# nekStab/nekStab_next

Measured on AMD Instinct MI355X. Metric: Arnoldi-step GB/s (achieved HBM) + Ritz-value rel-err, N=1e8 m=128, higher is better.
Workload: dtype f64

## Files before the change

### include/nekkrylov.h

```cpp
#ifndef NEKKRYLOV_H
#define NEKKRYLOV_H

#include <stddef.h>
#include <stdint.h>

#ifdef __cplusplus
extern "C" {
#endif

#define NKV_ABI_VERSION 3

#define NKV_TILE 4096
#define NKV_MAX_COLS 1024
#define NKV_ROT_MAX_OUT 256

#define NKV_OK 0
#define NKV_EINVAL 1
#define NKV_EHIP 2
#define NKV_ENAN 3
#define NKV_ESHAPE 4
#define NKV_ECALLBACK 5
#define NKV_EBREAKDOWN 6

#define NKV_TIME 0x1u
// ... 50 lines not shown
                     double* f, double* nrm2_dev, void* ws, unsigned flags, void* stream);
int nkv_block_update_dot(const nkv_layout* L, const double* w, const double* Q, int j, const double* h_dev,
                         double* f, double* hout_dev, void* ws, unsigned flags, void* stream);
int nkv_arnoldi_finish(const nkv_layout* L, const double* f, const double* nrm2_dev, double* q_out,
                       int j, const double* h1_dev, const double* h2_dev, double* hcol_dev,
                       unsigned flags, void* stream);

int nkv_combine(const nkv_layout* L, const double* Q, int k, const double* y_dev, double* out, unsigned flags,
                void* stream);
int nkv_normalize_store(const nkv_layout* L, const double* f, const double* nrm2_dev, double* q_next,
                        double* beta_dev, unsigned flags, void* stream);
int nkv_mgs2_step(const nkv_layout* L, const double* w, const double* Q, int j, double* f, double* q_out,
                  double* hcol_dev, void* ws, unsigned flags, void* stream);
int nkv_axpy_dot(const nkv_layout* L, const double* w, double* f, const double* alpha_dev, const double* qa,
                 const double* qb, double* out_dev, void* ws, unsigned flags, void* stream);

int nkv_block_dot2(const nkv_layout* L, const double* w, const double* Q, int j, const double* x,
                   const double* y, double* h_dev, void* ws, unsigned flags, void* stream);
int nkv_dcgs2_coef(int m, const double* hq_dev, const double* hw_dev, const double* nrm_prev_dev, double* H_dev,
                   int64_t ldh, double* coef_dev, void* ws, void* stream);
int nkv_dcgs2_update(const nkv_layout* L, const double* w, const double* Q, int m, const double* coef_dev,
                     double* qj, const double* win, double* fout, double* nrm2_dev, void* ws, unsigned flags,
                     void* stream);

int nkv_mgs_icwy_solve(int j, double* G, int64_t ldg, const double* grow, const double* b, double* x,
                       void* stream);

int nkv_gkl_coef(int side, int m, const double* hq_dev, const double* hw_dev, double* M_dev, int64_t ldm,
                 double* A_self, double* r_self, const double* A_other, const double* r_other, int64_t lda,
                 double* coef_dev, void* ws, void* stream);

typedef int (*nkv_matvec_fn)(void* user, const double* x, double* y, void* stream);
typedef int (*nkv_allreduce_fn)(void* user, double* buf, int n, void* stream);
size_t nkv_arnoldi_scratch_doubles(int m);
int nkv_arnoldi_dcgs2(const nkv_layout* L, const double* w, double* Q, int mstart, int mend, double* H_dev,
                      int64_t ldh, double* f, double* scratch_dev, void* ws, nkv_matvec_fn matvec, void* mv_user,
                      nkv_allreduce_fn allreduce, void* ar_user, unsigned flags, void* stream);

int nkv_gmres_dcgs2(const nkv_layout* L, const double* w, double* Q, int kmax, double beta, double tol2,
                    double* H_dev, int64_t ldh, double* f, double* scratch_dev, void* ws, nkv_matvec_fn matvec,
                    void* mv_user, nkv_allreduce_fn allreduce, void* ar_user, double* res_hist, int* k_out,
                    unsigned flags, void* stream);

int nkv_update_hessenberg(const nkv_layout* L, const double* w, const double* Q, int j, double* f, double* q_out,
                          double* hcol_dev, double* scratch_dev, void* ws, nkv_allreduce_fn allreduce, void* ar_user,
                          unsigned flags, void* stream);
// ... 4 lines not shown

int nkv_rotate(const nkv_layout* L, double* Q, int k, const double* V_dev, int ldv, void* stream);

int nkv_rotate_cols(const nkv_layout* L, double* Q, int k, const double* V_dev, int ldv, int n_out,
                    void* stream);

#define NKV_ROT_PATH_FEW 1
#define NKV_ROT_PATH_WIDE 2
#define NKV_ROT_PATH_STREAM 3
#define NKV_ROT_PATH_CHUNKED 4
int nkv_rotate_plan(const nkv_layout* L, int k, int ldv, int n_out, int* path, int* inst, int* wg_threads,
                    int* rows_per_tile);

#define NKV_STREAM_BLOCK_DOT 1
#define NKV_STREAM_BLOCK_UPDATE 2
#define NKV_STREAM_UPDATE_DOT 3
#define NKV_STREAM_BLOCK_DOT2 4
#define NKV_STREAM_DCGS2_UPDATE 5
#define NKV_STREAM_AXPY_DOT 6
#define NKV_STREAM_BLAS1 7
#define NKV_STREAM_OP_DIAG 8
#define NKV_STREAM_FINISH 9
#define NKV_STREAM_SPLIT 10
#define NKV_STREAM_LOOP_TILES 1
#define NKV_STREAM_LOOP_UNITS 2
typedef struct nkv_plan {
    int64_t kernel, pairs, nw, cpw, wg_threads, rows_per_tile, tiles, grid_x, grid_y, launches, band_tiles,
        last_grid_x, work_loop, units, fields_per_block, partial_slots, partial_cols;
} nkv_plan;
int nkv_stream_plan(const nkv_layout* L, int op, int j, unsigned flags, nkv_plan* plan);

int nkv_op_diag(const nkv_layout* L, const double* d, const double* x, double* y, double time_scale,
                void* stream);
int nkv_op_rot2(const nkv_layout* L, const double* c, const double* s, const double* d_rest,
                const double* x, double* y, int transpose, void* stream);
int nkv_op_cdiag(const nkv_layout* L, const double* cr, const double* ci, const double* x, double* y, int conj,
                 void* stream);

int nkv_wavemaker(const nkv_layout* L, const double* dRe, const double* dIm, const double* aRe, const double* aIm,
                  double* out, int ncomp, void* stream);
int nkv_gradm1(const nkv_layout* L, int lx1, int ldim, const double* D, const double* xm, const double* ym,
               const double* zm, const double* u, int nfld, int64_t u_stride, double* grad, int64_t g_stride,
               void* stream);
int nkv_bf_sensitivity(const nkv_layout* L, const double* dRe, const double* dIm, const double* aRe,
                       const double* aIm, const double* grad, double* out, int ncomp, void* stream);

// ... 149 lines not shown
```

### nekstab_next_amd/_lib.py

```python
from __future__ import annotations

import ctypes
import os
from ctypes import CFUNCTYPE, POINTER, Structure, c_char_p, c_double, c_int, c_int32, c_int64, c_size_t, c_uint, c_uint64, c_void_p

import torch

_HERE = os.path.dirname(os.path.abspath(__file__))
LIB_PATH = os.path.join(_HERE, "libnekkrylov.so")

NKV_ABI_VERSION = 3
NKV_TILE = 4096
NKV_MAX_COLS = 1024
NKV_ROT_MAX_OUT = 256
NKV_GS_MAX_FIELDS = 64
NKV_ROT_PATH_FEW, NKV_ROT_PATH_WIDE, NKV_ROT_PATH_STREAM, NKV_ROT_PATH_CHUNKED = 1, 2, 3, 4
(NKV_STREAM_BLOCK_DOT, NKV_STREAM_BLOCK_UPDATE, NKV_STREAM_UPDATE_DOT, NKV_STREAM_BLOCK_DOT2, NKV_STREAM_DCGS2_UPDATE,
 NKV_STREAM_AXPY_DOT, NKV_STREAM_BLAS1, NKV_STREAM_OP_DIAG, NKV_STREAM_FINISH, NKV_STREAM_SPLIT) = range(1, 11)
NKV_STREAM_LOOP_TILES, NKV_STREAM_LOOP_UNITS = 1, 2
NKV_OK, NKV_EINVAL, NKV_EHIP, NKV_ENAN, NKV_ESHAPE, NKV_ECALLBACK, NKV_EBREAKDOWN = 0, 1, 2, 3, 4, 5, 6
NKV_TIME = 0x1
NKV_ACCUMULATE = 0x2
NKV_OVERWRITE = 0x4
NKV_NORM2 = 0x8
NKV_TIME_DOT = 0x10
NKV_X_IS_LAST = 0x20
NKV_MGS2 = 0x40
NKV_MGS_ICWY = 0x100
NKV_MGS_LAGGED = 0x200
NKV_CHECK_BREAKDOWN = 0x80
NKV_SFD_MONITOR = 0x400
NKV_TDF_STORE = 0x800
NKV_BF_IMAG = 0x1000
NKV_BF_PERTURBATION = 0x2000
(NKV_VC_VORTICITY, NKV_VC_LAMBDA2, NKV_VC_Q, NKV_VC_DELTA, NKV_VC_SWIRLING, NKV_VC_OMEGA, NKV_VC_SYMMETRIC,
 NKV_VC_ASSYMETRIC, NKV_VC_LAMBDA_CI, NKV_VC_COUNT) = range(10)


class NkvError(RuntimeError):

    def __init__(self, code: int, where: str, msg: str):
        super().__init__(f"{where}: status {code}: {msg}")
# ... 35 lines not shown
_SIGNATURES = {
    "nkv_abi_version": (c_int, []),
    "nkv_layout_init": (c_int, [_L, c_int, c_int, c_int, c_int64, c_int64, c_int, c_int, c_int]),
    "nkv_last_error": (c_char_p, []),
    "nkv_device_info": (c_int, [POINTER(c_int), POINTER(c_int), POINTER(c_int64), c_char_p, c_int]),
    "nkv_workspace_bytes": (c_size_t, [_L, c_int]),
    "nkv_check_status": (c_int, [_P, _P]),
    "nkv_zero": (c_int, [_L, _P, c_uint, _P]),
    "nkv_copy": (c_int, [_L, _P, _P, c_uint, _P]),
    "nkv_scal": (c_int, [_L, _P, c_double, c_uint, _P]),
    "nkv_axpby": (c_int, [_L, _P, c_double, _P, c_double, c_uint, _P]),
    "nkv_sub3": (c_int, [_L, _P, _P, _P, c_uint, _P]),
    "nkv_axpy_dev": (c_int, [_L, _P, _P, c_double, _P, c_uint, _P]),
    "nkv_normalize_dev": (c_int, [_L, _P, _P, _P, c_uint, _P]),
    "nkv_dot": (c_int, [_L, _P, _P, _P, _P, _P, c_uint, _P]),
    "nkv_block_dot": (c_int, [_L, _P, _P, c_int, _P, _P, _P, c_uint, _P]),
    "nkv_block_update": (c_int, [_L, _P, _P, c_int, _P, _P, _P, _P, c_uint, _P]),
    "nkv_block_update_dot": (c_int, [_L, _P, _P, c_int, _P, _P, _P, _P, c_uint, _P]),
    "nkv_arnoldi_finish": (c_int, [_L, _P, _P, _P, c_int, _P, _P, _P, c_uint, _P]),
    "nkv_block_dot2": (c_int, [_L, _P, _P, c_int, _P, _P, _P, _P, c_uint, _P]),
    "nkv_dcgs2_coef": (c_int, [c_int, _P, _P, _P, _P, c_int64, _P, _P, _P]),
    "nkv_mgs_icwy_solve": (c_int, [c_int, _P, c_int64, _P, _P, _P, _P]),
    "nkv_dcgs2_update": (c_int, [_L, _P, _P, c_int, _P, _P, _P, _P, _P, _P, c_uint, _P]),
    "nkv_arnoldi_scratch_doubles": (c_size_t, [c_int]),
    "nkv_arnoldi_dcgs2": (c_int, [_L, _P, _P, c_int, c_int, _P, c_int64, _P, _P, _P, MATVEC_FN, _P, ALLREDUCE_FN, _P,
                                  c_uint, _P]),
    "nkv_update_hessenberg": (c_int, [_L, _P, _P, c_int, _P, _P, _P, _P, _P, ALLREDUCE_FN, _P, c_uint, _P]),
    "nkv_gmres_dcgs2": (c_int, [_L, _P, _P, c_int, c_double, c_double, _P, c_int64, _P, _P, _P, MATVEC_FN, _P,
                                ALLREDUCE_FN, _P, _P, _P, c_uint, _P]),
    "nkv_arnoldi_factorization": (c_int, [_L, _P, _P, c_int, c_int, _P, c_int64, _P, _P, _P, MATVEC_FN, _P,
                                          ALLREDUCE_FN, _P, c_uint, _P]),
    "nkv_combine": (c_int, [_L, _P, c_int, _P, _P, c_uint, _P]),
    "nkv_normalize_store": (c_int, [_L, _P, _P, _P, _P, c_uint, _P]),
    "nkv_mgs2_step": (c_int, [_L, _P, _P, c_int, _P, _P, _P, _P, c_uint, _P]),
    "nkv_axpy_dot": (c_int, [_L, _P, _P, _P, _P, _P, _P, _P, c_uint, _P]),
    "nkv_rotate": (c_int, [_L, _P, c_int, _P, c_int, _P]),
    "nkv_rotate_cols": (c_int, [_L, _P, c_int, _P, c_int, c_int, _P]),
    "nkv_rotate_plan": (c_int, [_L, c_int, c_int, c_int, POINTER(c_int), POINTER(c_int), POINTER(c_int),
                                POINTER(c_int)]),
    "nkv_stream_plan": (c_int, [_L, c_int, c_int, c_uint, POINTER(nkv_plan)]),
    "nkv_op_diag": (c_int, [_L, _P, _P, _P, c_double, _P]),
    "nkv_op_rot2": (c_int, [_L, _P, _P, _P, _P, _P, c_int, _P]),
    "nkv_op_cdiag": (c_int, [_L, _P, _P, _P, _P, c_int, _P]),
    "nkv_fill_hash": (c_int, [_L, _P, c_uint64, c_int64, c_int64, _P]),
    "nkv_mth_rand_add": (c_int, [_L, c_int, c_int, c_int, c_int64, _P, _P, _P, c_double, c_double, c_double, _P, _P]),
    "nkv_group_average": (c_int, [c_int64, _P, _P, _P, _P]),
# ... 110 lines not shown
```

### nekstab_next_amd/arnoldi.py

```python
from __future__ import annotations

import numpy as np
import torch

from . import _lib
from ._lib import NKV_NORM2, NKV_TIME, NKV_TIME_DOT, NKV_X_IS_LAST
from .operators import LinearOperator
from .vector import Basis, NekContext, NekVector


class HessenbergDev:

    def __init__(self, ctx: NekContext, k: int):
        self.ctx, self.k = ctx, k
        self.t = torch.zeros((k, k + 1), dtype=torch.float64, device=ctx.device)

    def col_ptr(self, c: int) -> int:
        return self.t[c].data_ptr()

    def download(self) -> np.ndarray:
        return np.asfortranarray(self.t.detach().cpu().numpy().T)

    def upload(self, H: np.ndarray) -> None:
        self.t.copy_(torch.as_tensor(np.ascontiguousarray(np.asarray(H, dtype=np.float64).T)).to(self.ctx.device))
# ... 60 lines not shown
    elif mode == "mgs2":
        ctx.call("nkv_dot", w, f.ptr, Q.col_ptr(0), h1[0:1].data_ptr(), ws, tf, st)
        ctx.comm.allreduce_(h1[0:1])
        fl = NKV_TIME | (NKV_TIME_DOT if tf else 0)
        for p, h in enumerate((h1, h2)):
            for i in range(j):
                last = i + 1 == j
                qn = Q.col_ptr(i + 1) if not last else (Q.col_ptr(0) if p == 0 else None)
                out = h[i + 1:i + 2] if not last else (h2[0:1] if p == 0 else nrm)
                ctx.call("nkv_axpy_dot", w, f.ptr, h[i:i + 1].data_ptr(), Q.col_ptr(i), qn, out.data_ptr(), ws, fl,
                         st)
                ctx.comm.allreduce_(out)
    else:
        raise ValueError(f"unknown orthogonalisation mode {mode!r}")
    if ctx.timer:
        ctx.timer.begin("finish")
    ctx.call("nkv_arnoldi_finish", f.ptr, nrm.data_ptr(), out_ptr, j, h1.data_ptr(), h2.data_ptr(),
             hcol_ptr, 0, st)
    if ctx.timer:
        ctx.timer.end("finish", 16.0 * ctx.layout.N)


def _dcgs2_step(ctx: NekContext, Q: Basis, Hd: HessenbergDev, j: int, f: NekVector, first: bool,
                nrm2: torch.Tensor | None = None) -> None:
    w, ws, st = ctx.w.data_ptr(), ctx.ws.data_ptr(), ctx.stream
    lay, tm = ctx.layout, ctx.timer
    tf = NKV_TIME if ctx.time_in_dot else 0
    m = j - 1
    h = ctx.hd[: 2 * j]
    hp, cp = h.data_ptr(), ctx.coef.data_ptr()
    u = Q.col_ptr(m)
    if tm:
        tm.begin("block_dot2")
    ctx.call("nkv_block_dot2", w, Q.ptr, j, u, f.ptr, hp, ws, tf | NKV_X_IS_LAST, st)
    if tm:
        tm.end("block_dot2", 8.0 * ((j - 1) * lay.N_w + 2 * lay.N_w + lay.n_v))
    ctx.comm.allreduce_(h)
    nprev = None if first else (nrm2.data_ptr() if nrm2 is not None else hp + 8 * m)
    ctx.call_nl("nkv_dcgs2_coef", m, hp, hp + 8 * j, nprev, Hd.t.data_ptr(), Hd.k + 1, cp, ws, st)
    if tm:
        tm.begin("dcgs2_update")
    ctx.call("nkv_dcgs2_update", w, Q.ptr, m, cp, u, f.ptr, Q.col_ptr(j), None if nrm2 is None else nrm2.data_ptr(),
             ws, NKV_TIME | (NKV_TIME_DOT if tf else 0), st)
    if tm:
        tm.end("dcgs2_update", 8.0 * (m * lay.N + 4 * lay.N) + (0.0 if nrm2 is None else 8.0 * lay.n_v))
    if nrm2 is not None:
        ctx.comm.allreduce_(nrm2)


def _dcgs2_close(ctx: NekContext, Q: Basis, Hd: HessenbergDev, m: int) -> None:
    w, ws, st = ctx.w.data_ptr(), ctx.ws.data_ptr(), ctx.stream
    lay, tm = ctx.layout, ctx.timer
    tf = NKV_TIME if ctx.time_in_dot else 0
    h, coef = ctx.hd[: m + 1], ctx.coef
    u = Q.col_ptr(m)
    if tm:
        tm.begin("block_dot")
    ctx.call("nkv_block_dot", w, Q.ptr, m + 1, u, h.data_ptr(), ws, tf, st)
    if tm:
        tm.end("block_dot", 8.0 * ((m + 1) * lay.N_w + lay.N_w + lay.n_v))
    ctx.comm.allreduce_(h)
    ctx.call_nl("nkv_dcgs2_coef", m, h.data_ptr(), None, h.data_ptr() + 8 * m, Hd.t.data_ptr(), Hd.k + 1,
                coef.data_ptr(), ws, st)
    if tm:
        tm.begin("block_update")
    ctx.call("nkv_block_update", w, Q.ptr, m, h.data_ptr(), u, None, ws, NKV_TIME, st)
    if tm:
        tm.end("block_update", 8.0 * (m * lay.N + 2 * lay.N))
    ctx.call("nkv_normalize_dev", u, coef[2 * m + 3:].data_ptr(), None, 0, st)


def _icwy_gram(ctx: NekContext, Q: Basis, mstart: int) -> torch.Tensor:
    ldg = ctx.max_cols + 1
    G = getattr(ctx, "_icwy_G", None)
    if G is None:
        G = ctx._icwy_G = torch.zeros((ldg, ldg), dtype=torch.float64, device=ctx.device)
    w, ws, st = ctx.w.data_ptr(), ctx.ws.data_ptr(), ctx.stream
    tf = NKV_TIME if ctx.time_in_dot else 0
    for i in range(1, mstart - 1):
        ctx.call("nkv_block_dot", w, Q.ptr, i, Q.col_ptr(i), G[i].data_ptr(), ws, tf, st)
        ctx.comm.allreduce_(G[i, :i])
    return G

# ... 174 lines not shown
        raise errors[0]
    _lib.check(rc, entry)


def arnoldi_factorization(ctx: NekContext, op: LinearOperator, Q: Basis, Hd: HessenbergDev, mstart: int,
                          mend: int, f: NekVector | None = None, mode: str = "cgs2", transpose: bool = False,
                          on_step=None) -> None:
    if mend < mstart:
        return
    if Q.k < mend + 1:
        raise ValueError("basis too small")
    if f is None:
        f = ctx.vector()
    if mode == "dcgs2-native":
        if on_step is None:
            if mend > ctx.max_cols or mend + 1 > Hd.k + 1:
                raise ValueError(f"step {mend} exceeds max_cols {ctx.max_cols} / H size {Hd.k}")
            _dcgs2_native(ctx, op, Q, Hd, mstart, mend, f, transpose)
            return
        mode = "dcgs2"
    if mode == "dcgs2" and on_step is not None:
        if mend > ctx.max_cols or mend + 1 > Hd.k + 1:
            raise ValueError(f"step {mend} exceeds max_cols {ctx.max_cols} / H size {Hd.k}")
        for mstep in range(mstart, mend + 1):
            (op.rmatvec if transpose else op.matvec)(Q[mstep - 1], f)
            _dcgs2_step(ctx, Q, Hd, mstep, f, first=(mstep == mstart))
            if mstep > mstart:
                on_step(mstep - 1)
        _dcgs2_close(ctx, Q, Hd, mend)
        on_step(mend)
        return
    if mode == "mgs2-lagged-native":
        if on_step is None:
            if mend > ctx.max_cols or mend + 1 > Hd.k + 1:
                raise ValueError(f"step {mend} exceeds max_cols {ctx.max_cols} / H size {Hd.k}")
            _dcgs2_native(ctx, op, Q, Hd, mstart, mend, f, transpose, entry="nkv_arnoldi_factorization",
                          flags=_lib.NKV_MGS_LAGGED)
            return
        mode = "mgs2-lagged"
    if mode == "mgs2-lagged":
        if mend > ctx.max_cols or mend + 1 > Hd.k + 1:
            raise ValueError(f"step {mend} exceeds max_cols {ctx.max_cols} / H size {Hd.k}")
        _lagged_factorization(ctx, op, Q, Hd, mstart, mend, f, transpose, on_step)
        return
    if mode == "mgs2-icwy-native":
        if on_step is None:
            if mend > ctx.max_cols or mend + 1 > Hd.k + 1:
                raise ValueError(f"step {mend} exceeds max_cols {ctx.max_cols} / H size {Hd.k}")
            _dcgs2_native(ctx, op, Q, Hd, mstart, mend, f, transpose, entry="nkv_arnoldi_factorization",
                          flags=_lib.NKV_MGS_ICWY)
            return
        mode = "mgs2-icwy"
    if mode == "mgs2-icwy":
        if mend > ctx.max_cols or mend + 1 > Hd.k + 1:
            raise ValueError(f"step {mend} exceeds max_cols {ctx.max_cols} / H size {Hd.k}")
        G = _icwy_gram(ctx, Q, mstart)
        for mstep in range(mstart, mend + 1):
            (op.rmatvec if transpose else op.matvec)(Q[mstep - 1], f)
            _icwy_step(ctx, Q, Hd, mstep, f, G)
            if on_step is not None:
                on_step(mstep)
        return
    if mode in ("cgs2-native", "mgs2-native") and on_step is None:
        if mend > ctx.max_cols or mend + 1 > Hd.k + 1:
            raise ValueError(f"step {mend} exceeds max_cols {ctx.max_cols} / H size {Hd.k}")
        _dcgs2_native(ctx, op, Q, Hd, mstart, mend, f, transpose, entry="nkv_arnoldi_factorization",
                      flags=_lib.NKV_MGS2 if mode == "mgs2-native" else 0)
        return
    if mode == "dcgs2" and on_step is None:
        if mend > ctx.max_cols or mend + 1 > Hd.k + 1:
            raise ValueError(f"step {mend} exceeds max_cols {ctx.max_cols} / H size {Hd.k}")
        for mstep in range(mstart, mend + 1):
            (op.rmatvec if transpose else op.matvec)(Q[mstep - 1], f)
            _dcgs2_step(ctx, Q, Hd, mstep, f, first=(mstep == mstart))
        _dcgs2_close(ctx, Q, Hd, mend)
        return
    if mode == "dcgs2":
        mode = "cgs2"
    for mstep in range(mstart, mend + 1):
        x = Q[mstep - 1]
        (op.rmatvec if transpose else op.matvec)(x, f)
        update_hessenberg_matrix(ctx, Q, mstep, f, Hd, mode)
        if on_step is not None:
            on_step(mstep)


class FactorizationGraph:

    def __init__(self, ctx: NekContext, op: LinearOperator, Q: Basis, Hd: HessenbergDev, f: NekVector,
                 mode: str = "cgs2"):
        self.ctx, self.op, self.Q, self.Hd, self.f, self.mode = ctx, op, Q, Hd, f, mode
        self.graphs = {}

    HOST_SYNC_MODES = ("mgs2-lagged", "mgs2-lagged-native")

    def usable(self) -> bool:
        return self.ctx.comm.world == 1 and self.mode not in self.HOST_SYNC_MODES

# ... 17 lines not shown
```

### nekstab_next_amd/csrc/core.hip

```cpp
#include "nkv_internal.h"

namespace nkvi {

thread_local char g_err[512] = "";

int fail(int code, const char* fmt, ...) {
    va_list ap;
    va_start(ap, fmt);
    vsnprintf(g_err, sizeof(g_err), fmt, ap);
    va_end(ap);
    return code;
}

int device_cus() {
    static int cus[64] = {0};
    int dev = 0;
    if (hipGetDevice(&dev) != hipSuccess || dev < 0 || dev >= 64) return 256;
    if (!cus[dev]) {
        int n = 0;
        cus[dev] = (hipDeviceGetAttribute(&n, hipDeviceAttributeMultiprocessorCount, dev) == hipSuccess && n > 0)
                       ? n : 256;
    }
    return cus[dev];
}
// ... 122 lines not shown
            if (bmax > kMaxBlocks) bmax = kMaxBlocks;
            p.grid_x = bmax / p.grid_y;
            if (p.grid_x > p.tiles) p.grid_x = p.tiles;
            if (p.grid_x < 1) p.grid_x = 1;
            p.work_loop = NKV_STREAM_LOOP_TILES;
            p.units = p.tiles;
            p.band_tiles = p.tiles > 0 ? p.tiles : 1;
            p.launches = p.tiles > 0 ? 1 : 0;
            p.last_grid_x = p.grid_x;
            p.partial_slots = p.tiles > 0 ? p.grid_x * p.grid_y : 0;
            p.partial_cols = two ? 2 * j : j;
            break;
        }
        case NKV_STREAM_BLOCK_UPDATE: {
            if (j < 0) return fail(NKV_EINVAL, "j=%d < 0", j);
            set_tile_grid(&p, L, large ? NKV_PAIRS : NKV_PAIRS_SMALL, j <= NKV_UPD_SMALL_J ? 4 * kMaxBlocks : kMaxBlocks);
            set_bands(&p, NKV_UPD_ROUNDS, true);
            if (flags & NKV_NORM2) {
                p.partial_slots = p.grid_x;
                p.partial_cols = 1;
            }
            break;
        }
        case NKV_STREAM_UPDATE_DOT: {
            if (j < 1 || j > NKV_MAX_COLS) return fail(NKV_EINVAL, "j=%d outside 1..%d", j, NKV_MAX_COLS);
            if (j > 256 || rows >= (int64_t)1 << 29) {
                p.kernel = NKV_STREAM_SPLIT;
                break;
            }
            constexpr int NW = NKV_FUSE_NW;
            p.nw = j <= NKV_FUSE_SMALL_J ? 4 : (j <= NW * 16 ? NW : 16);
            p.cpw = (j + p.nw - 1) / p.nw;
            p.pairs = 1;
            p.wg_threads = p.nw * 64;
            p.rows_per_tile = kFuseRows;
            p.tiles = rows / kFuseRows;
            const int64_t gcap = (j >= NKV_FUSE_MID_LO && j <= NKV_FUSE_MID_HI) ? NKV_FUSE_G_MID : NKV_FUSE_G;
            p.grid_x = p.tiles < gcap ? p.tiles : gcap;
            if (p.grid_x < 1) p.grid_x = 1;
            p.grid_y = 1;
            p.work_loop = NKV_STREAM_LOOP_TILES;
            p.units = p.tiles;
            p.fields_per_block = 1;
            set_bands(&p, NKV_FUSE_ROUNDS, true);
            p.partial_slots = p.grid_x;
            p.partial_cols = j;
            break;
        }
        case NKV_STREAM_DCGS2_UPDATE: {
            if (j < 0) return fail(NKV_EINVAL, "m=%d < 0", j);
            set_tile_grid(&p, L, large ? NKV_DC_PAIRS : NKV_PAIRS_SMALL, NKV_DC_G < kMaxBlocks ? NKV_DC_G : kMaxBlocks);
            if (!(flags & NKV_NORM2)) {
                set_bands(&p, NKV_DC_ROUNDS, true);
                break;
            }
            set_bands(&p, 0, true);
            const int64_t tpf = L->sv / p.rows_per_tile;
            if (!(tpf < p.grid_x && j >= 8)) {
                p.work_loop = NKV_STREAM_LOOP_UNITS;
                p.units = tpf + (p.tiles - tpf * L->n_wf);
            }
            p.partial_slots = p.grid_x;
            p.partial_cols = 1;
            break;
        }
        case NKV_STREAM_AXPY_DOT: {
            set_tile_grid(&p, L, NKV_PAIRS_SMALL, kMaxBlocks);
            set_bands(&p, NKV_AXD_ROUNDS, true);
            p.partial_slots = p.tiles > 0 ? p.grid_x : 0;
// ... 39 lines not shown
```

### nekstab_next_amd/csrc/drivers.hip

```cpp
#include "nkv_internal.h"

#include <vector>

extern "C" {

static size_t icwy_scratch_doubles(int m) { return (size_t)(4 * (m + 1) + 2) + (size_t)(m + 1) * (size_t)(m + 1); }
size_t nkv_arnoldi_scratch_doubles(int m) {
    const size_t base = (size_t)(2 * (m + 1) + 4 * m + 16), icwy = icwy_scratch_doubles(m);
    return base > icwy ? base : icwy;
}

static constexpr double kBreakdownTol = 1e-8;

static int check_breakdown(const double* H_dev, int64_t ldh, int c0, int c1, void* ws, void* stream) {
    if (c0 < 0) c0 = 0;
    if (c1 <= c0) return NKV_OK;
    hipStream_t st = S(stream);
    const size_t n = (size_t)ldh * (size_t)(c1 - c0);
    double* h = static_cast<double*>(malloc(n * sizeof(double)));
    if (!h) return fail(NKV_EINVAL, "breakdown check: host allocation of %zu doubles failed", n);
    int flag = 0;
    hipError_t e = hipMemcpyAsync(h, H_dev + (int64_t)c0 * ldh, n * sizeof(double), hipMemcpyDeviceToHost, st);
    if (e == hipSuccess) e = hipMemcpyAsync(&flag, nan_flag_of(ws), sizeof(int), hipMemcpyDeviceToHost, st);
    if (e == hipSuccess) e = hipStreamSynchronize(st);
// ... 26 lines not shown
                      int64_t ldh, double* f, double* scratch_dev, void* ws, nkv_matvec_fn matvec, void* mv_user,
                      nkv_allreduce_fn allreduce, void* ar_user, unsigned flags, void* stream) {
    CHECK(check_layout(L));
    CHECK(check_ptr(Q, "Q"));
    CHECK(check_ptr(f, "f"));
    if (!matvec) return fail(NKV_EINVAL, "matvec callback is NULL");
    if (!H_dev || !scratch_dev) return fail(NKV_EINVAL, "H/scratch is NULL");
    if (mstart < 1 || mend > NKV_MAX_COLS) return fail(NKV_EINVAL, "steps %d..%d outside 1..%d", mstart, mend, NKV_MAX_COLS);
    if (mend < mstart) return NKV_OK;
    if (ldh < mend + 1) return fail(NKV_EINVAL, "ldh=%lld < mend+1=%d", (long long)ldh, mend + 1);
    const unsigned tf = (flags & NKV_TIME_DOT) ? NKV_TIME : 0u;
    double* hd = scratch_dev;
    double* coef = scratch_dev + 2 * (mend + 1);
    auto col = [L, Q](int c) { return Q + (int64_t)c * L->ld; };
    for (int j = mstart; j <= mend; ++j) {
        const int m = j - 1;
        double* u = col(m);
        int rc = matvec(mv_user, u, f, stream);
        if (rc != 0) return fail(NKV_ECALLBACK, "matvec callback returned %d at step %d", rc, j);
        CHECK(nkv_block_dot2(L, w, Q, j, u, f, hd, ws, tf | NKV_X_IS_LAST, stream));
        if (allreduce && (rc = allreduce(ar_user, hd, 2 * j, stream)) != 0)
            return fail(NKV_ECALLBACK, "allreduce callback returned %d at step %d", rc, j);
        CHECK(nkv_dcgs2_coef(m, hd, hd + j, j == mstart ? nullptr : hd + m, H_dev, ldh, coef, ws, stream));
        CHECK(nkv_dcgs2_update(L, w, Q, m, coef, u, f, col(j), nullptr, ws, NKV_TIME, stream));
    }
    const int m = mend;
    double* u = col(m);
    CHECK(nkv_block_dot(L, w, Q, m + 1, u, hd, ws, tf, stream));
    if (allreduce) {
        const int rc = allreduce(ar_user, hd, m + 1, stream);
        if (rc != 0) return fail(NKV_ECALLBACK, "allreduce callback returned %d (closing step)", rc);
    }
    CHECK(nkv_dcgs2_coef(m, hd, nullptr, hd + m, H_dev, ldh, coef, ws, stream));
    CHECK(nkv_block_update(L, w, Q, m, hd, u, nullptr, ws, NKV_TIME, stream));
    CHECK(nkv_normalize_dev(L, u, coef + 2 * m + 3, nullptr, 0, stream));
    return (flags & NKV_CHECK_BREAKDOWN) ? check_breakdown(H_dev, ldh, mstart - 1, mend, ws, stream) : NKV_OK;
}

int nkv_gmres_dcgs2(const nkv_layout* L, const double* w, double* Q, int kmax, double beta, double tol2,
                    double* H_dev, int64_t ldh, double* f, double* scratch_dev, void* ws, nkv_matvec_fn matvec,
                    void* mv_user, nkv_allreduce_fn allreduce, void* ar_user, double* res_hist, int* k_out,
                    unsigned flags, void* stream) {
    CHECK(check_layout(L));
    CHECK(check_ptr(Q, "Q"));
    CHECK(check_ptr(f, "f"));
    CHECK(check_ptr(w, "w"));
    CHECK(check_ptr(ws, "ws"));
    if (!matvec) return fail(NKV_EINVAL, "matvec callback is NULL");
    if (!H_dev || !scratch_dev || !res_hist || !k_out) return fail(NKV_EINVAL, "H/scratch/res_hist/k_out is NULL");
    if (kmax < 1 || kmax + 1 > NKV_MAX_COLS) return fail(NKV_EINVAL, "kmax=%d outside 1..%d", kmax, NKV_MAX_COLS - 1);
    if (ldh < kmax + 1) return fail(NKV_EINVAL, "ldh=%lld < kmax+1=%d", (long long)ldh, kmax + 1);
// ... 324 lines not shown
```

### nekstab_next_amd/csrc/gram_schmidt.hip

```cpp
#include "nkv_internal.h"

namespace {

template <bool OVERWRITE, bool NORM, int kPairs>
__global__ __launch_bounds__(kThreads) void k_block_update(const double* __restrict__ Q, int64_t ld,
                                                           int j, const double* __restrict__ h,
                                                           double* __restrict__ f,
                                                           const double* __restrict__ w, int64_t sv,
                                                           int tiles_per_field, int tiles_w,
                                                           int tiles_total, int64_t time_off,
                                                           int do_time,
                                                           double* __restrict__ partials, int t_lo,
                                                           int acc_part) {
    constexpr int kTile = kThreads * kPairs * 2;
    __shared__ double lds4[4];
    if (do_time && blockIdx.x == 0 && threadIdx.x < 64) {
        double s = 0.0;
        for (int c = threadIdx.x; c < j; c += 64) s = fma(Q[time_off + (int64_t)c * ld], h[c], s);
        s = wave_sum(s);
        if (threadIdx.x == 0) f[time_off] = OVERWRITE ? s : f[time_off] - s;
    }
    double nrm = 0.0;
    for (int t = t_lo + blockIdx.x; t < tiles_total; t += gridDim.x) {
        const int64_t r0 = (int64_t)t * kTile + 2 * threadIdx.x;
// ... 517 lines not shown
    const int n_wf = tiles_per_field > 0 ? tiles_w / tiles_per_field : 0;
    const int n_units = tiles_per_field + (tiles_total - tiles_w);
    for (int u = blockIdx.x; u < n_units; u += gridDim.x) {
        if (u < tiles_per_field) {
            double2 wv[kPairs];
#pragma unroll
            for (int k = 0; k < kPairs; ++k) wv[k] = ld2(w + (int64_t)u * kTile + 2 * threadIdx.x + k * 2 * kThreads);
            for (int fi = 0; fi < n_wf; ++fi) {
                dcgs2_tile<kPairs>(Q, ld, m, a, x, rinv, yc, sc, qj, win, f,
                                   (int64_t)(fi * tiles_per_field + u) * kTile + 2 * threadIdx.x, af);
#pragma unroll
                for (int k = 0; k < kPairs; ++k) {
                    nrm = fma(wv[k].x * af[k].x, af[k].x, nrm);
                    nrm = fma(wv[k].y * af[k].y, af[k].y, nrm);
                }
            }
        } else {
            dcgs2_tile<kPairs>(Q, ld, m, a, x, rinv, yc, sc, qj, win, f,
                               (int64_t)(tiles_w + u - tiles_per_field) * kTile + 2 * threadIdx.x, af);
        }
    }
    nrm = block_sum(nrm, lds4);
    if (threadIdx.x == 0) partials[blockIdx.x] = nrm;
}

template <int P>
int launch_block_update_p(const nkv_layout* L, const nkv_plan& p, const double* w, const double* Q, int j,
                          const double* h_dev, double* f, double* part, unsigned flags, hipStream_t st) {
    const bool over = (flags & NKV_OVERWRITE) != 0;
    const bool norm = (flags & NKV_NORM2) != 0;
    const int tpf = (int)(L->sv / p.rows_per_tile);
    const int tiles_w = tpf * L->n_wf;
    const int tiles_total = (int)p.tiles;
    const int64_t T = rows_of(L);
    const int dt = (flags & NKV_TIME) ? 1 : 0;
    auto kern = over ? (norm ? k_block_update<true, true, P> : k_block_update<true, false, P>)
                     : (norm ? k_block_update<false, true, P> : k_block_update<false, false, P>);
    for (int64_t i = 0; i < p.launches; ++i) {
        const int lo = (int)(i * p.band_tiles);
        const int hi = lo + p.band_tiles < tiles_total ? (int)(lo + p.band_tiles) : tiles_total;
        const int64_t gb = i + 1 == p.launches ? p.last_grid_x : p.grid_x;
        hipLaunchKernelGGL(kern, dim3((unsigned)gb), dim3(kThreads), 0, st, Q, L->ld, j, h_dev, f, w, L->sv, tpf, tiles_w,
                           hi, T, lo == 0 ? dt : 0, part, lo, lo == 0 ? 0 : 1);
        NKV_LAUNCHED();
    }
    return NKV_OK;
// ... 215 lines not shown
    const int tpf = (int)(L->sv / p.rows_per_tile);
    const int tiles_w = tpf * L->n_wf;
    const int tiles_total = (int)p.tiles;
    const int g = (int)p.grid_x;
    const int64_t T = rows_of(L);
    const int dt = (flags & NKV_TIME) ? 1 : 0;
    double* part = partials_of(ws);
    auto kern = large ? (nrm2_dev ? k_dcgs2_update<NKV_DC_PAIRS, true> : k_dcgs2_update<NKV_DC_PAIRS, false>)
                      : (nrm2_dev ? k_dcgs2_update<NKV_PAIRS_SMALL, true> : k_dcgs2_update<NKV_PAIRS_SMALL, false>);
    for (int64_t i = 0; i < p.launches; ++i) {
        const int lo = (int)(i * p.band_tiles);
        const int hi = lo + p.band_tiles < tiles_total ? (int)(lo + p.band_tiles) : tiles_total;
        const int64_t gb = i + 1 == p.launches ? p.last_grid_x : p.grid_x;
        hipLaunchKernelGGL(kern, dim3((unsigned)gb), dim3(kThreads), 0, st, Q, L->ld, m, coef_dev, qj, win, fout, w, L->sv,
                           tpf, tiles_w, tiles_total, T, lo == 0 ? dt : 0, part, lo, hi);
        NKV_LAUNCHED();
    }
    if (!nrm2_dev) return NKV_OK;
    const bool tdot = (flags & NKV_TIME_DOT) && L->rank0;
    CHECK(launch_reduce_cols(1, part, g, nrm2_dev, tdot ? fout + T : nullptr, (int64_t)0, tdot ? fout + T : nullptr, nullptr, 1 << 30, nan_flag_of(ws), st));
    return NKV_OK;
}

int nkv_combine(const nkv_layout* L, const double* Q, int k, const double* y_dev, double* out, unsigned flags,
                void* stream) {
    return nkv_block_update(L, nullptr, Q, k, y_dev, out, nullptr, nullptr,
                            (flags & ~(unsigned)NKV_NORM2) | NKV_OVERWRITE, stream);
}

}
```

### nekstab_next_amd/vector.py

```python
from __future__ import annotations

import ctypes

import numpy as np
import torch

from . import _lib
from ._lib import NKV_OVERWRITE, NKV_TIME
from .comm import Comm
from .layout import NekLayout


def _ptr(t: torch.Tensor) -> int:
    return t.data_ptr()


class NekContext:

    def __init__(self, layout: NekLayout, weights=None, comm: Comm | None = None, max_cols: int = 256,
                 device: torch.device | int | None = None, time_in_dot: bool = False):
        if not 1 <= max_cols < _lib.NKV_MAX_COLS:
            raise ValueError(f"max_cols={max_cols} outside 1..{_lib.NKV_MAX_COLS - 1}")
        _lib.require_gpu()
        self.comm = comm if comm is not None else Comm()
# ... 250 lines not shown
    t_keep = ctx.scal[6:7]
    t_keep.copy_(q.storage[to:to + 1])
    ctx.call("nkv_normalize_dev", q.ptr, _ptr(out), _ptr(beta), 0, ctx.stream)
    q.storage[to:to + 1].copy_(t_keep)
    return float(beta.item())


ROTATE_PATHS = {_lib.NKV_ROT_PATH_FEW: "few", _lib.NKV_ROT_PATH_WIDE: "wide", _lib.NKV_ROT_PATH_STREAM: "stream",
                _lib.NKV_ROT_PATH_CHUNKED: "chunked"}


def rotate_plan(layout, k: int, n_out: int, ldv: int | None = None) -> tuple[str, int, int, int]:
    L = layout.c_struct() if isinstance(layout, NekLayout) else layout
    out = [ctypes.c_int(0) for _ in range(4)]
    rc = _lib.load().nkv_rotate_plan(ctypes.byref(L), int(k), int(k if ldv is None else ldv), int(n_out),
                                     *[ctypes.byref(o) for o in out])
    _lib.check(rc, "nkv_rotate_plan")
    return ROTATE_PATHS[out[0].value], out[1].value, out[2].value, out[3].value


STREAM_OPS = {"block_dot": _lib.NKV_STREAM_BLOCK_DOT, "block_update": _lib.NKV_STREAM_BLOCK_UPDATE,
              "update_dot": _lib.NKV_STREAM_UPDATE_DOT, "block_dot2": _lib.NKV_STREAM_BLOCK_DOT2,
              "dcgs2_update": _lib.NKV_STREAM_DCGS2_UPDATE, "axpy_dot": _lib.NKV_STREAM_AXPY_DOT,
              "blas1": _lib.NKV_STREAM_BLAS1, "op_diag": _lib.NKV_STREAM_OP_DIAG, "finish": _lib.NKV_STREAM_FINISH}
_STREAM_KERNELS = {**{v: k for k, v in STREAM_OPS.items()}, _lib.NKV_STREAM_SPLIT: "split"}
_STREAM_LOOPS = {0: None, _lib.NKV_STREAM_LOOP_TILES: "tiles", _lib.NKV_STREAM_LOOP_UNITS: "units"}


class StreamPlan(dict):

    __getattr__ = dict.__getitem__


def stream_plan(layout, op: str, j: int = 1, flags: int = 0) -> StreamPlan:
    L = layout.c_struct() if isinstance(layout, NekLayout) else layout
    p = _lib.nkv_plan()
    _lib.check(_lib.load().nkv_stream_plan(ctypes.byref(L), STREAM_OPS[op], int(j), int(flags), ctypes.byref(p)),
               "nkv_stream_plan")
    out = StreamPlan((name, int(getattr(p, name))) for name, _ in p._fields_)
    out["kernel"] = _STREAM_KERNELS[out["kernel"]]
    out["work_loop"] = _STREAM_LOOPS[out["work_loop"]]
    return out


__all__ = [
    "NekContext", "NekVector", "ComplexNekVector", "Basis", "k_dot", "k_norm", "k_normalize", "k_cmult",
    "k_add2", "k_sub2", "k_sub3", "k_zero", "k_copy", "k_matmul", "combine", "NKV_NORM2",
# ... 4 lines not shown
```

Baseline: 6718.

## Fuse final DCGS2 update with closing block dot to skip a basis pass

On the last Arnoldi step of a cycle, a new kernel applies the DCGS2 update and also accumulates the weighted dot products of the new residual against all basis columns, the updated column and itself. The closing step then no longer launches a separate block_dot, which would re-read the whole basis. The saving happens once per restart cycle rather than on every step. In exchange the code gains a large set of template instantiations and a more complex shared-memory reduction. When m is above 256 it falls back to the split path.

```diff
diff --git a/include/nekkrylov.h b/include/nekkrylov.h
--- a/include/nekkrylov.h
+++ b/include/nekkrylov.h
@@ -96,6 +96,9 @@
 int nkv_dcgs2_update(const nkv_layout* L, const double* w, const double* Q, int m, const double* coef_dev,
                      double* qj, const double* win, double* fout, double* nrm2_dev, void* ws, unsigned flags,
                      void* stream);
+int nkv_dcgs2_update_close(const nkv_layout* L, const double* w, const double* Q, int m, const double* coef_dev,
+                           double* qj, const double* win, double* fout, double* h_dev, void* ws, unsigned flags,
+                           void* stream);
 
 int nkv_mgs_icwy_solve(int j, double* G, int64_t ldg, const double* grow, const double* b, double* x,
                        void* stream);
@@ -146,6 +149,7 @@
 #define NKV_STREAM_OP_DIAG 8
 #define NKV_STREAM_FINISH 9
 #define NKV_STREAM_SPLIT 10
+#define NKV_PLAN_DCGS2_UPDATE_CLOSE 12
 #define NKV_STREAM_LOOP_TILES 1
 #define NKV_STREAM_LOOP_UNITS 2
 typedef struct nkv_plan {
diff --git a/nekstab_next_amd/_lib.py b/nekstab_next_amd/_lib.py
--- a/nekstab_next_amd/_lib.py
+++ b/nekstab_next_amd/_lib.py
@@ -18,6 +18,7 @@
 (NKV_STREAM_BLOCK_DOT, NKV_STREAM_BLOCK_UPDATE, NKV_STREAM_UPDATE_DOT, NKV_STREAM_BLOCK_DOT2, NKV_STREAM_DCGS2_UPDATE,
  NKV_STREAM_AXPY_DOT, NKV_STREAM_BLAS1, NKV_STREAM_OP_DIAG, NKV_STREAM_FINISH, NKV_STREAM_SPLIT) = range(1, 11)
 NKV_STREAM_LOOP_TILES, NKV_STREAM_LOOP_UNITS = 1, 2
+NKV_PLAN_DCGS2_UPDATE_CLOSE = 12
 NKV_OK, NKV_EINVAL, NKV_EHIP, NKV_ENAN, NKV_ESHAPE, NKV_ECALLBACK, NKV_EBREAKDOWN = 0, 1, 2, 3, 4, 5, 6
 NKV_TIME = 0x1
 NKV_ACCUMULATE = 0x2
@@ -99,6 +100,7 @@
     "nkv_dcgs2_coef": (c_int, [c_int, _P, _P, _P, _P, c_int64, _P, _P, _P]),
     "nkv_mgs_icwy_solve": (c_int, [c_int, _P, c_int64, _P, _P, _P, _P]),
     "nkv_dcgs2_update": (c_int, [_L, _P, _P, c_int, _P, _P, _P, _P, _P, _P, c_uint, _P]),
+    "nkv_dcgs2_update_close": (c_int, [_L, _P, _P, c_int, _P, _P, _P, _P, _P, _P, c_uint, _P]),
     "nkv_arnoldi_scratch_doubles": (c_size_t, [c_int]),
     "nkv_arnoldi_dcgs2": (c_int, [_L, _P, _P, c_int, c_int, _P, c_int64, _P, _P, _P, MATVEC_FN, _P, ALLREDUCE_FN, _P,
                                   c_uint, _P]),
diff --git a/nekstab_next_amd/arnoldi.py b/nekstab_next_amd/arnoldi.py
--- a/nekstab_next_amd/arnoldi.py
+++ b/nekstab_next_amd/arnoldi.py
@@ -106,7 +106,7 @@
 
 
 def _dcgs2_step(ctx: NekContext, Q: Basis, Hd: HessenbergDev, j: int, f: NekVector, first: bool,
-                nrm2: torch.Tensor | None = None) -> None:
+                nrm2: torch.Tensor | None = None, last: bool = False) -> bool:
     w, ws, st = ctx.w.data_ptr(), ctx.ws.data_ptr(), ctx.stream
     lay, tm = ctx.layout, ctx.timer
     tf = NKV_TIME if ctx.time_in_dot else 0
@@ -124,25 +124,32 @@
     ctx.call_nl("nkv_dcgs2_coef", m, hp, hp + 8 * j, nprev, Hd.t.data_ptr(), Hd.k + 1, cp, ws, st)
     if tm:
         tm.begin("dcgs2_update")
-    ctx.call("nkv_dcgs2_update", w, Q.ptr, m, cp, u, f.ptr, Q.col_ptr(j), None if nrm2 is None else nrm2.data_ptr(),
-             ws, NKV_TIME | (NKV_TIME_DOT if tf else 0), st)
-    if tm:
-        tm.end("dcgs2_update", 8.0 * (m * lay.N + 4 * lay.N) + (0.0 if nrm2 is None else 8.0 * lay.n_v))
+    fused = last and nrm2 is None
+    if fused:
+        ctx.call("nkv_dcgs2_update_close", w, Q.ptr, m, cp, u, f.ptr, Q.col_ptr(j), hp, ws,
+                 NKV_TIME | (NKV_TIME_DOT if tf else 0), st)
+    else:
+        ctx.call("nkv_dcgs2_update", w, Q.ptr, m, cp, u, f.ptr, Q.col_ptr(j), None if nrm2 is None else nrm2.data_ptr(),
+                 ws, NKV_TIME | (NKV_TIME_DOT if tf else 0), st)
+    if tm:
+        tm.end("dcgs2_update", 8.0 * (m * lay.N + 4 * lay.N) + (0.0 if nrm2 is None and not fused else 8.0 * lay.n_v))
     if nrm2 is not None:
         ctx.comm.allreduce_(nrm2)
-
-
-def _dcgs2_close(ctx: NekContext, Q: Basis, Hd: HessenbergDev, m: int) -> None:
+    return fused
+
+
+def _dcgs2_close(ctx: NekContext, Q: Basis, Hd: HessenbergDev, m: int, have_dots: bool = False) -> None:
     w, ws, st = ctx.w.data_ptr(), ctx.ws.data_ptr(), ctx.stream
     lay, tm = ctx.layout, ctx.timer
     tf = NKV_TIME if ctx.time_in_dot else 0
     h, coef = ctx.hd[: m + 1], ctx.coef
     u = Q.col_ptr(m)
-    if tm:
-        tm.begin("block_dot")
-    ctx.call("nkv_block_dot", w, Q.ptr, m + 1, u, h.data_ptr(), ws, tf, st)
-    if tm:
-        tm.end("block_dot", 8.0 * ((m + 1) * lay.N_w + lay.N_w + lay.n_v))
+    if not have_dots:
+        if tm:
+            tm.begin("block_dot")
+        ctx.call("nkv_block_dot", w, Q.ptr, m + 1, u, h.data_ptr(), ws, tf, st)
+        if tm:
+            tm.end("block_dot", 8.0 * ((m + 1) * lay.N_w + lay.N_w + lay.n_v))
     ctx.comm.allreduce_(h)
     ctx.call_nl("nkv_dcgs2_coef", m, h.data_ptr(), None, h.data_ptr() + 8 * m, Hd.t.data_ptr(), Hd.k + 1,
                 coef.data_ptr(), ws, st)
@@ -363,12 +370,13 @@
     if mode == "dcgs2" and on_step is not None:
         if mend > ctx.max_cols or mend + 1 > Hd.k + 1:
             raise ValueError(f"step {mend} exceeds max_cols {ctx.max_cols} / H size {Hd.k}")
+        have_dots = False
         for mstep in range(mstart, mend + 1):
             (op.rmatvec if transpose else op.matvec)(Q[mstep - 1], f)
-            _dcgs2_step(ctx, Q, Hd, mstep, f, first=(mstep == mstart))
+            have_dots = _dcgs2_step(ctx, Q, Hd, mstep, f, first=(mstep == mstart), last=(mstep == mend))
             if mstep > mstart:
                 on_step(mstep - 1)
-        _dcgs2_close(ctx, Q, Hd, mend)
+        _dcgs2_close(ctx, Q, Hd, mend, have_dots)
         on_step(mend)
         return
     if mode == "mgs2-lagged-native":
@@ -411,10 +419,11 @@
     if mode == "dcgs2" and on_step is None:
         if mend > ctx.max_cols or mend + 1 > Hd.k + 1:
             raise ValueError(f"step {mend} exceeds max_cols {ctx.max_cols} / H size {Hd.k}")
+        have_dots = False
         for mstep in range(mstart, mend + 1):
             (op.rmatvec if transpose else op.matvec)(Q[mstep - 1], f)
-            _dcgs2_step(ctx, Q, Hd, mstep, f, first=(mstep == mstart))
-        _dcgs2_close(ctx, Q, Hd, mend)
+            have_dots = _dcgs2_step(ctx, Q, Hd, mstep, f, first=(mstep == mstart), last=(mstep == mend))
+        _dcgs2_close(ctx, Q, Hd, mend, have_dots)
         return
     if mode == "dcgs2":
         mode = "cgs2"
diff --git a/nekstab_next_amd/csrc/core.hip b/nekstab_next_amd/csrc/core.hip
--- a/nekstab_next_amd/csrc/core.hip
+++ b/nekstab_next_amd/csrc/core.hip
@@ -168,8 +168,12 @@
             }
             break;
         }
-        case NKV_STREAM_UPDATE_DOT: {
-            if (j < 1 || j > NKV_MAX_COLS) return fail(NKV_EINVAL, "j=%d outside 1..%d", j, NKV_MAX_COLS);
+        case NKV_STREAM_UPDATE_DOT:
+        case NKV_PLAN_DCGS2_UPDATE_CLOSE: {
+            const bool close = op == NKV_PLAN_DCGS2_UPDATE_CLOSE;
+            if (close && (j < 0 || j + 2 > NKV_MAX_COLS))
+                return fail(NKV_EINVAL, "m=%d outside 0..%d", j, NKV_MAX_COLS - 2);
+            if (!close && (j < 1 || j > NKV_MAX_COLS)) return fail(NKV_EINVAL, "j=%d outside 1..%d", j, NKV_MAX_COLS);
             if (j > 256 || rows >= (int64_t)1 << 29) {
                 p.kernel = NKV_STREAM_SPLIT;
                 break;
@@ -177,6 +181,7 @@
             constexpr int NW = NKV_FUSE_NW;
             p.nw = j <= NKV_FUSE_SMALL_J ? 4 : (j <= NW * 16 ? NW : 16);
             p.cpw = (j + p.nw - 1) / p.nw;
+            if (p.cpw < 1) p.cpw = 1;
             p.pairs = 1;
             p.wg_threads = p.nw * 64;
             p.rows_per_tile = kFuseRows;
@@ -190,7 +195,7 @@
             p.fields_per_block = 1;
             set_bands(&p, NKV_FUSE_ROUNDS, true);
             p.partial_slots = p.grid_x;
-            p.partial_cols = j;
+            p.partial_cols = close ? j + 2 : j;
             break;
         }
         case NKV_STREAM_DCGS2_UPDATE: {
diff --git a/nekstab_next_amd/csrc/drivers.hip b/nekstab_next_amd/csrc/drivers.hip
--- a/nekstab_next_amd/csrc/drivers.hip
+++ b/nekstab_next_amd/csrc/drivers.hip
@@ -72,11 +72,15 @@
         if (allreduce && (rc = allreduce(ar_user, hd, 2 * j, stream)) != 0)
             return fail(NKV_ECALLBACK, "allreduce callback returned %d at step %d", rc, j);
         CHECK(nkv_dcgs2_coef(m, hd, hd + j, j == mstart ? nullptr : hd + m, H_dev, ldh, coef, ws, stream));
-        CHECK(nkv_dcgs2_update(L, w, Q, m, coef, u, f, col(j), nullptr, ws, NKV_TIME, stream));
+        if (j < mend) {
+            CHECK(nkv_dcgs2_update(L, w, Q, m, coef, u, f, col(j), nullptr, ws, NKV_TIME, stream));
+        } else {
+            CHECK(nkv_dcgs2_update_close(L, w, Q, m, coef, u, f, col(j), hd, ws, NKV_TIME | (flags & NKV_TIME_DOT),
+                                         stream));
+        }
     }
     const int m = mend;
     double* u = col(m);
-    CHECK(nkv_block_dot(L, w, Q, m + 1, u, hd, ws, tf, stream));
     if (allreduce) {
         const int rc = allreduce(ar_user, hd, m + 1, stream);
         if (rc != 0) return fail(NKV_ECALLBACK, "allreduce callback returned %d (closing step)", rc);
diff --git a/nekstab_next_amd/csrc/gram_schmidt.hip b/nekstab_next_amd/csrc/gram_schmidt.hip
--- a/nekstab_next_amd/csrc/gram_schmidt.hip
+++ b/nekstab_next_amd/csrc/gram_schmidt.hip
@@ -563,6 +563,123 @@
     }
     nrm = block_sum(nrm, lds4);
     if (threadIdx.x == 0) partials[blockIdx.x] = nrm;
+}
+
+template <int NW, int CPW>
+__global__ __launch_bounds__(NW * 64, 4) void k_dcgs2_update_dot(const double* __restrict__ Q, int64_t ld, int m,
+                                                               const double* __restrict__ coef,
+                                                               double* __restrict__ qj,
+                                                               const double* __restrict__ win,
+                                                               double* __restrict__ f,
+                                                               const double* __restrict__ w, int64_t sv,
+                                                               int64_t tiles_per_field, int64_t tiles_w,
+                                                               int64_t tiles_total, int64_t time_off,
+                                                               int do_time, double* __restrict__ partials,
+                                                               int B, int64_t t_lo, int acc_part) {
+    __shared__ double2 part[2][NW][2][64];
+    __shared__ double2 cf[NW * CPW];
+    const int wv = __builtin_amdgcn_readfirstlane(threadIdx.x >> 6);
+    const int lane = threadIdx.x & 63;
+    const double* x = coef;
+    const double* a = coef + 2 * m + 5;
+    const double rinv = coef[2 * m + 1], yc = coef[2 * m + 2], sc = coef[2 * m + 4];
+    const double wsc = sc * rinv;
+    for (int c = threadIdx.x; c < NW * CPW; c += NW * 64) cf[c] = c < m ? make_double2(-a[c], -x[c]) : make_double2(0.0, 0.0);
+    if (do_time && blockIdx.x == 0 && wv == 0) {
+        double s1 = 0.0, s2 = 0.0;
+        for (int c = lane; c < m; c += 64) {
+            const double qt = Q[time_off + (int64_t)c * ld];
+            s1 = fma(qt, a[c], s1);
+            s2 = fma(qt, x[c], s2);
+        }
+        s1 = wave_sum(s1);
+        s2 = wave_sum(s2);
+        if (lane == 0) {
+            const double qb = (qj[time_off] * sc - s1) * rinv;
+            qj[time_off] = qb;
+            f[time_off] = win[time_off] * wsc - s2 - qb * yc;
+        }
+    }
+    __syncthreads();
+    const double* qcol[CPW];
+#pragma unroll
+    for (int i = 0; i < CPW; ++i) {
+        const int c = wv + NW * i;
+        qcol[i] = Q + (int64_t)(c < m ? c : 0) * ld;
+    }
+    double acc[CPW];
+#pragma unroll
+    for (int i = 0; i < CPW; ++i) acc[i] = 0.0;
+    double acc_q = 0.0, acc_u = 0.0;
+    int buf = 0;
+    double2 q[CPW];
+    for (int64_t t = t_lo + blockIdx.x; t < tiles_total; t += gridDim.x, buf ^= 1) {
+        const uint32_t r = (uint32_t)(t * kFuseRows) + 2u * lane;
+        const uint32_t rb = r * 8u;
+#pragma unroll
+        for (int i = 0; i < CPW - 1; ++i) q[i] = ldq(at_b(qcol[i], rb));
+        q[CPW - 1] = (wv + NW * (CPW - 1) < m) ? ldq(at_b(qcol[CPW - 1], rb)) : make_double2(0.0, 0.0);
+        double2 sa = make_double2(0.0, 0.0), sx = make_double2(0.0, 0.0);
+        if (wv == 0) {
+            const double2 uv = ld2(at_b(qj, rb)), fv = ld2(at_b(win, rb));
+            sa = make_double2(uv.x * sc, uv.y * sc);
+            sx = make_double2(fv.x * wsc, fv.y * wsc);
+        }
+        const bool weighted = t < tiles_w;
+        const double2 ww = weighted ? ld2(at_b(w, (r - (uint32_t)((t / tiles_per_field) * sv)) * 8u)) : make_double2(0.0, 0.0);
+#pragma unroll
+        for (int i = 0; i < CPW; ++i) {
+            const double2 c2 = cf[wv + NW * i];
+            sa.x = fma(c2.x, q[i].x, sa.x);
+            sa.y = fma(c2.x, q[i].y, sa.y);
+            sx.x = fma(c2.y, q[i].x, sx.x);
+            sx.y = fma(c2.y, q[i].y, sx.y);
+        }
+        part[buf][wv][0][lane] = sa;
+        part[buf][wv][1][lane] = sx;
+        __syncthreads();
+        double2 ta = part[buf][0][0][lane], tx = part[buf][0][1][lane];
+#pragma unroll 2
+        for (int k = 1; k < NW; ++k) {
+            const double2 pa = part[buf][k][0][lane], px = part[buf][k][1][lane];
+            ta.x += pa.x;
+            ta.y += pa.y;
+            tx.x += px.x;
+            tx.y += px.y;
+        }
+        const double2 qb = make_double2(ta.x * rinv, ta.y * rinv);
+        const double2 un = make_double2(fma(-yc, qb.x, tx.x), fma(-yc, qb.y, tx.y));
+        if (wv == 0) {
+            st2p(qj, (int64_t)r, qb);
+            st2p(f, (int64_t)r, un);
+        }
+        if (weighted) {
+            const double da = ww.x * un.x, db = ww.y * un.y;
+#pragma unroll
+            for (int i = 0; i < CPW; ++i) acc[i] = fma(q[i].y, db, fma(q[i].x, da, acc[i]));
+            if (wv == NW - 1) {
+                acc_q = fma(qb.y, db, fma(qb.x, da, acc_q));
+                acc_u = fma(un.y, db, fma(un.x, da, acc_u));
+            }
+        }
+    }
+    auto put = [&](int c, double v) {
+        double* p = partials + (int64_t)c * B + blockIdx.x;
+        *p = acc_part ? *p + v : v;
+    };
+#pragma unroll
+    for (int i = 0; i < CPW; ++i) {
+        const int c = wv + NW * i;
+        const double v = wave_sum(acc[i]);
+        if (lane == 0 && c < m) put(c, v);
+    }
+    if (wv == NW - 1) {
+        const double vq = wave_sum(acc_q), vu = wave_sum(acc_u);
+        if (lane == 0) {
+            put(m, vq);
+            put(m + 1, vu);
+        }
+    }
 }
 
 template <int P>
@@ -824,6 +941,90 @@
     return NKV_OK;
 }
 
+int nkv_dcgs2_update_close(const nkv_layout* L, const double* w, const double* Q, int m, const double* coef_dev,
+                           double* qj, const double* win, double* fout, double* h_dev, void* ws, unsigned flags,
+                           void* stream) {
+    CHECK(check_layout(L));
+    CHECK(check_ptr(w, "w"));
+    CHECK(check_ptr(Q, "Q"));
+    CHECK(check_ptr(qj, "qj"));
+    CHECK(check_ptr(win, "win"));
+    CHECK(check_ptr(fout, "fout"));
+    CHECK(check_ptr(ws, "ws"));
+    nkv_plan p;
+    CHECK(nkv_stream_plan(L, NKV_PLAN_DCGS2_UPDATE_CLOSE, m, flags, &p));
+    if (!coef_dev || !h_dev) return fail(NKV_EINVAL, "coef/h_dev is NULL");
+    if (qj != Q + (int64_t)m * L->ld || fout != Q + (int64_t)(m + 1) * L->ld)
+        return fail(NKV_EINVAL, "dcgs2_update_close: qj / fout are not columns m / m+1 of Q");
+    hipStream_t st = S(stream);
+    if (p.kernel == NKV_STREAM_SPLIT) {
+        CHECK(nkv_dcgs2_update(L, w, Q, m, coef_dev, qj, win, fout, nullptr, ws, flags, stream));
+        return launch_block_dot(L, w, Q, L->ld, m + 2, fout, h_dev, ws, (flags & NKV_TIME_DOT) ? NKV_TIME : 0u, st);
+    }
+    const int64_t tiles_total = p.tiles;
+    const int64_t tpf = L->sv / kFuseRows;
+    const int64_t tiles_w = tpf * L->n_wf;
+    const int B = (int)p.partial_slots;
+    const int64_t T = rows_of(L);
+    const int dt = (flags & NKV_TIME) ? 1 : 0;
+    double* part = partials_of(ws);
+#define NKV_CLOSE(NW, CPW)                                                                                       \
+    for (int64_t i = 0; i < p.launches; ++i) {                                                                   \
+        const int64_t lo = i * p.band_tiles;                                                                     \
+        const int64_t hi = lo + p.band_tiles < tiles_total ? lo + p.band_tiles : tiles_total;                    \
+        const int64_t gb = i + 1 == p.launches ? p.last_grid_x : p.grid_x;                                       \
+        hipLaunchKernelGGL((k_dcgs2_update_dot<NW, CPW>), dim3((unsigned)gb), dim3(NW * 64), 0, st, Q, L->ld, m,  \
+                           coef_dev, qj, win, fout, w, L->sv, tpf, tiles_w, hi, T, lo == 0 ? dt : 0, part, B, lo, \
+                           lo == 0 ? 0 : 1);                                                                     \
+    }
+    constexpr int NW = NKV_FUSE_NW;
+    const int cpw = (int)p.cpw;
+    if (p.nw == 4 && NW != 4) {
+        switch (cpw) {
+            case 1: NKV_CLOSE(4, 1); break;
+            case 2: NKV_CLOSE(4, 2); break;
+            case 3: NKV_CLOSE(4, 3); break;
+            default: NKV_CLOSE(4, 4); break;
+        }
+    } else if (p.nw == NW) {
+        switch (cpw) {
+            case 1: NKV_CLOSE(NW, 1); break;
+            case 2: NKV_CLOSE(NW, 2); break;
+            case 3: NKV_CLOSE(NW, 3); break;
+            case 4: NKV_CLOSE(NW, 4); break;
+            case 5: NKV_CLOSE(NW, 5); break;
+            case 6: NKV_CLOSE(NW, 6); break;
+            case 7: NKV_CLOSE(NW, 7); break;
+            case 8: NKV_CLOSE(NW, 8); break;
+            case 9: NKV_CLOSE(NW, 9); break;
+            case 10: NKV_CLOSE(NW, 10); break;
+            case 11: NKV_CLOSE(NW, 11); break;
+            case 12: NKV_CLOSE(NW, 12); break;
+            case 13: NKV_CLOSE(NW, 13); break;
+            case 14: NKV_CLOSE(NW, 14); break;
+            case 15: NKV_CLOSE(NW, 15); break;
+            default: NKV_CLOSE(NW, 16); break;
+        }
+    } else {
+        switch (cpw) {
+            case 9: NKV_CLOSE(16, 9); break;
+            case 10: NKV_CLOSE(16, 10); break;
+            case 11: NKV_CLOSE(16, 11); break;
+            case 12: NKV_CLOSE(16, 12); break;
+            case 13: NKV_CLOSE(16, 13); break;
+            case 14: NKV_CLOSE(16, 14); break;
+            case 15: NKV_CLOSE(16, 15); break;
+            default: NKV_CLOSE(16, 16); break;
+        }
+    }
+#undef NKV_CLOSE
+    NKV_LAUNCHED();
+    const bool tdot = (flags & NKV_TIME_DOT) && L->rank0;
+    CHECK(launch_reduce_cols(m + 2, part, B, h_dev, tdot ? Q + T : nullptr, L->ld, tdot ? fout + T : nullptr, nullptr,
+                             1 << 30, nan_flag_of(ws), st));
+    return NKV_OK;
+}
+
 int nkv_combine(const nkv_layout* L, const double* Q, int k, const double* y_dev, double* out, unsigned flags,
                 void* stream) {
     return nkv_block_update(L, nullptr, Q, k, y_dev, out, nullptr, nullptr,
diff --git a/nekstab_next_amd/vector.py b/nekstab_next_amd/vector.py
--- a/nekstab_next_amd/vector.py
+++ b/nekstab_next_amd/vector.py
@@ -296,7 +296,8 @@
 STREAM_OPS = {"block_dot": _lib.NKV_STREAM_BLOCK_DOT, "block_update": _lib.NKV_STREAM_BLOCK_UPDATE,
               "update_dot": _lib.NKV_STREAM_UPDATE_DOT, "block_dot2": _lib.NKV_STREAM_BLOCK_DOT2,
               "dcgs2_update": _lib.NKV_STREAM_DCGS2_UPDATE, "axpy_dot": _lib.NKV_STREAM_AXPY_DOT,
-              "blas1": _lib.NKV_STREAM_BLAS1, "op_diag": _lib.NKV_STREAM_OP_DIAG, "finish": _lib.NKV_STREAM_FINISH}
+              "blas1": _lib.NKV_STREAM_BLAS1, "op_diag": _lib.NKV_STREAM_OP_DIAG, "finish": _lib.NKV_STREAM_FINISH,
+              "dcgs2_update_close": _lib.NKV_PLAN_DCGS2_UPDATE_CLOSE}
 _STREAM_KERNELS = {**{v: k for k, v in STREAM_OPS.items()}, _lib.NKV_STREAM_SPLIT: "split"}
 _STREAM_LOOPS = {0: None, _lib.NKV_STREAM_LOOP_TILES: "tiles", _lib.NKV_STREAM_LOOP_UNITS: "units"}
 
```

After: 6699. About the same (-0.3%).
